# facebookresearch/omni3d

Measured on AMD Instinct MI355X. Metric: images/sec train DLA34_FPN b=4/GPU, higher is better.
Workload: dtype f32; 1 GPU; cubercnn_DLA34_FPN train step, batch 4/GPU, synthetic Omni3D 512x512 (8 GT/img), fwd+10 losses+bwd+allreduce+divergence guard+SGD, random-init weights; global_batch=4, image=512x512, parallelism=dp1 (flat-bucket RCCL all-reduce)

## Files before the change

include/omni3d_hip.h:

```cpp
#ifndef OMNI3D_HIP_H
#define OMNI3D_HIP_H

#ifdef __cplusplus
extern "C" {
#endif


int omni_iou_box3d(const float* boxes1, int N, const float* boxes2, int M, const int* valid1, float* vol,
                   float* iou, int* overflow, void* stream);

int omni_iou_box3d_pairs(const float* boxes1, const float* boxes2, const int* idx1, const int* idx2,
                         long long npairs, const int* valid1, float* vol, float* iou, int* overflow,
                         void* stream);

int omni_iou_box3d_pairs_algo(const float* boxes1, const float* boxes2, const int* idx1, const int* idx2,
                              long long npairs, const int* valid1, float* vol, float* iou, int* overflow,
                              int lanes_per_pair, void* stream);

int omni_box3d_validity(const float* boxes, int N, float eps_coplanar, float eps_nonzero, int* valid,
                        int* counts, void* stream);

int omni_nms3d(const float* verts, const float* score, const int* cls, const int* count, int B, int S, float iou_thr,
               int class_agnostic, float eps_coplanar, float eps_nonzero, float* iou, int* keep, int* order, int* new_count,
               int* overflow, void* stream);
// ... 266 lines not shown
int omni_cuboid_corners(const float* box3d, const float* R, int n, float* verts, void* stream);

int omni_conv2d_fwd_stats(const float* x, const float* w, float* out, int N, int H, int W, int C, int K, int R, int S,
                          int stride, int pad, int ldx, int ldo, float* stats, int stats_rows, int* nblk_out, void* stream);
int omni_wino_out_stats(const float* M, float* y, int N, int H, int W, int K, int tile, float* stats, int stats_rows,
                        int* nblk_out, void* stream);
int omni_wino_out_bn_bwd_stats(const float* M, float* y, int N, int H, int W, int K, int tile, const float* bn_x,
                               const float* mean_rstd, const float* scale_shift, float* stats, int stats_rows, int* nblk_out,
                               void* stream);
int omni_stem_conv_fwd_stats(const float* x, const float* w, float* out, int N, int H, int W, int C, int K, int R, int ldx,
                             int ldo, float* stats, int stats_rows, int* nblk_out, void* stream);

int omni_gemm_engine(const float* A, const float* B, float* C, const float* bias, int form, int batch, int M, int N, int K,
                     int lda, int ldb, int ldc, long long stride_a, long long stride_b, long long stride_c, int splits,
                     int relu, int accumulate, int tile, int workgroups, void* stream);
int omni_gemm_engine_det(const float* A, const float* B, float* C, const float* bias, int form, int batch, int M, int N, int K,
                         int lda, int ldb, int ldc, long long stride_a, long long stride_b, long long stride_c, int splits,
                         int relu, int accumulate, int tile, int workgroups, float* ws, long long ws_floats, int* ctr, int n_ctr,
                         long long* plan, void* stream);

int omni_transpose2d(const float* src, float* dst, int rows, int cols, void* stream);

int omni_det_scores(const float* pred, int ld, const float* rois, const int* count, const int* image_hw, int B, int P, int K,
                    float wx, float wy, float ww, float wh, float score_thresh, float* scores, float* probs, float* boxes,
                    void* stream);
int omni_det_nms_boxes(const float* boxes, const float* vals, const int* idx, int B, int PK, int K, int cap, float* nms_boxes,
                       int* valid, void* stream);
int omni_det_compact(const int* keep, const int* valid, const float* vals, const int* idx, const float* boxes, int B, int PK,
                     int K, int cap, int topk, float* out_box, float* out_score, int* out_cls, int* out_roi, int* out_count,
                     void* stream);

int omni_resize_bilinear_u8(const unsigned char* src, unsigned char* dst, unsigned char* tmp, int planes, int H, int W,
                            int HO, int WO, const int* bounds_h, const int* kk_h, int ksize_h, const int* bounds_v,
                            const int* kk_v, int ksize_v, int flip, void* stream);
int omni_pil_bilinear_coeffs(int in_size, int out_size, int* bounds, int* kk, int ksize, void* stream);
int omni_crop_resize_u8(const unsigned char* src, unsigned char* dst, unsigned char* tmp, int planes, int H, int W, int x0, int y0,
                        int ch, int cw, int HO, int WO, const int* bounds_h, const int* kk_h, int ksize_h, const int* bounds_v,
                        const int* kk_v, int ksize_v, int flip, void* stream);
int omni_color_jitter_u8(unsigned char* img, int H, int W, int wb, int wc, int ws, int c_red, unsigned long long* sum, void* stream);
int omni_warp_homography_u8(const unsigned char* src, unsigned char* dst, int planes, int H, int W, int HO, int WO, const double* m,
                            const unsigned char* fill, void* stream);


int omni_sgd_step(float* param, const float* grad, float* momentum_buf, long long n, float lr, float momentum,
                  float dampening, float weight_decay, int nesterov, int first_step, float grad_scale,
                  const float* skip_flag, void* stream);
int omni_adam_step(float* param, const float* grad, float* exp_avg, float* exp_avg_sq, float* max_exp_avg_sq, long long n, float lr,
                   float beta1, float beta2, float eps, float weight_decay, int decoupled, const float* step, float grad_scale,
                   const float* skip_flag, void* stream);
int omni_adam_tick(float* step, const float* skip_flag, void* stream);
int omni_clip_norm_partials(const float* grad, const long long* tiles, int ntiles, float norm_type, double* partial, void* stream);
int omni_clip_norm_coef(const double* partial, const long long* ptab, int nparams, float norm_type, float max_norm, float grad_scale,
                        float* norm, float* coef, void* stream);
int omni_sgd_step_clipped(float* param, const float* grad, float* momentum_buf, const long long* tiles, int t0, int t1, int clip_mode,
                          const float* coef, float clip_value, float lr, float momentum, float dampening, float weight_decay,
                          int nesterov, int first_step, float grad_scale, const float* skip_flag, void* stream);
int omni_adam_step_clipped(float* param, const float* grad, float* exp_avg, float* exp_avg_sq, float* max_exp_avg_sq,
                           const long long* tiles, int t0, int t1, int clip_mode, const float* coef, float clip_value, float lr,
                           float beta1, float beta2, float eps, float weight_decay, int decoupled, const float* step,
                           float grad_scale, const float* skip_flag, void* stream);
int omni_guard_pre(float* vec, int n, void* stream);
int omni_guard_post(float* vec, int n, int world, float stabilize, float half_period, float tolerance, float gamma, float* state,
                    float* skip, float* out, void* stream);
int omni_scale_vec(const void* src, int src_f64, int stride, const double* coef, const void* denom, double denom_min, int n, float* out,
                   void* stream);
int omni_sum_vectors(const void* const* vecs, const int* lens, int nvec, int nfirst, float* out, void* stream);
int omni_guard_gather(const void* const* scalars, int n, float* vec, void* stream);
int omni_bump_counters(const void* const* counters, int n, long long delta, void* stream);
int omni_zero(void* p, long long nbytes, void* stream);
int omni_nonfinite_any(const float* grad, long long n, float* flag, void* stream);

int omni_relu_bwd(const float* dy, const float* y, float* dz, long long n, void* stream);
int omni_bias_grad(const float* dy, int P, int C, float* db, double* ws, int accumulate, void* stream);

int omni_maxpool3s2_fwd(const float* x, float* y, int N, int H, int W, int C, void* stream);
int omni_maxpool3s2_bwd(const float* x, const float* dy, float* dx, int N, int H, int W, int C, void* stream);

int omni_wino_in(const float* x, float* V, int N, int H, int W, int C, int tile, void* stream);
int omni_wino_out(const float* M, const float* bias, float* y, int N, int H, int W, int K, int relu, int tile, void* stream);
int omni_wino_dy(const float* dy, float* dM, int N, int H, int W, int K, int tile, void* stream);
int omni_wino_weights_multi(const void* const* g, const void* const* U, const void* const* U_flip, const int* K, const int* C,
                            const int* tile, int n, void* stream);
int omni_wino_dy_in(const float* dy, float* dM, float* Vd, int N, int H, int W, int K, int tile, void* stream);
int omni_wino_weights(const float* g, float* U , float* U_flip , int K, int C, int tile, void* stream);
int omni_wino_dweights(const float* dU, float* dg, int K, int C, int accumulate, int tile, void* stream);
int omni_wino_dweights_multi(const void* const* dU, const void* const* dg, const int* K, const int* C, const int* tile, int n,
                             void* stream);
int omni_gemm_batched_fwd_algo(const float* x, const float* w, float* out, int batch, int M, int C, int K, int algo,
                               int workgroups, void* stream);
int omni_gemm_batched_wgrad_algo(const float* x, const float* dy, float* dw, int batch, int M, int C, int K, int algo,
                                 void* stream);
int omni_gemm_batched_wgrad_det(const float* x, const float* dy, float* dw, int batch, int M, int C, int K, int algo, float* ws,
                                long long ws_floats, int* ctr, int n_ctr, long long* plan, void* stream);
int omni_gemm_batched_wgrad_multi(const void* const* x, const void* const* dy, const void* const* dw, const int* batch, const int* M,
                                  const int* C, const int* K, int n, float* ws, long long ws_floats, int* ctr, int n_ctr,
                                  long long* plan, void* stream);

int omni_stem_conv_fwd(const float* x, const float* w, float* out, int N, int H, int W, int C, int K, int R, int ldx, int ldo,
                       void* stream);
int omni_stem_conv_dgrad(const float* dy, const float* w, float* dx, int N, int H, int W, int C, int K, int R, int lddy, int lddx,
                         void* stream);
int omni_stem_conv_s2_dgrad(const float* dy, const float* w, float* dx, int N, int H, int W, int C, int K, int R, int lddy, int lddx,
                            void* stream);
int omni_stem_conv_wgrad(const float* x, const float* dy, float* dw, int N, int H, int W, int C, int K, int R, int ldx, int lddy,
                         int accumulate, void* stream);
int omni_stem_conv_wgrad_det(const float* x, const float* dy, float* dw, int N, int H, int W, int C, int K, int R, int ldx, int lddy,
                             int accumulate, float* ws, long long ws_floats, long long* plan, void* stream);
int omni_stem_conv_fwd_cw(const float* x, const float* w, int cw, float* out, int N, int H, int W, int C, int K, int R, int ldx, int ldo,
                          float* stats, int stats_rows, int* nblk_out, void* stream);
int omni_stem_conv_wgrad_det_cw(const float* x, const float* dy, float* dw, int cw, int N, int H, int W, int C, int K, int R, int ldx,
                                int lddy, int accumulate, float* ws, long long ws_floats, long long* plan, void* stream);
int omni_stem_conv_s2_wgrad(const float* x, const float* dy, float* dw, int N, int H, int W, int C, int K, int R, int ldx, int lddy,
                            int accumulate, int deterministic, float* ws, long long ws_floats, long long* plan, void* stream);

int omni_eval_match(const float* ious, const long long* iou_off, const int* dt_off, const int* gt_off, const int* gt_ignore,
                    const float* gt_range, const float* dt_range, const float* areas, const double* thrs, int ngroups, int A,
                    int T, int sumD, int sumG, int max_gt, int* dt_match, int* gt_match, unsigned char* dt_ignore, int* gt_order,
                    unsigned char* gt_ig, void* stream);

int omni_eval_accumulate(const int* order, const int* cat_off, const int* rank, const double* score, const int* dt_match,
                         const unsigned char* dt_ignore, const int* npig, const int* has_e, const double* rec_thrs,
                         const int* max_dets, int K, int A, int M, int T, int R, int sumD, double* precision, double* recall,
                         double* scores, void* stream);

int omni_eval_accumulate_par_workspace(int K, int A, int M, int T, int sumD, int block, long long* bytes);
int omni_eval_accumulate_par(const int* order, const int* cat_off, const int* rank, const double* score, const int* dt_match,
                             const unsigned char* dt_ignore, const int* npig, const int* has_e, const double* rec_thrs,
                             const int* max_dets, int K, int A, int M, int T, int R, int sumD, int block, void* workspace,
                             long long workspace_bytes, double* precision, double* recall, double* scores, void* stream);

int omni_eval_bootstrap_counts(const int* grp_off, const int* grp_img, const int* grp_npig, const int* weights, int max_weight, int K,
                               int A, int G, int sumG, int B, int I, int* npig_b, int* has_e_b, void* stream);
int omni_eval_bootstrap(const int* order, const int* cat_off, const int* rank, const int* dt_match, const unsigned char* dt_ignore,
                        const int* det_img, const int* weights, int max_weight, const int* npig_b, const int* has_e_b,
                        const double* rec_thrs, const int* max_dets, int K, int A, int M, int T, int R, int sumD, int B, int I,
                        double* ap, double* ar, void* stream);

int omni_eval_error_types(const float* sim, const long long* sim_off, const int* dt_off, const int* gt_off, const int* dt_cat,
                          const unsigned char* dt_matched, const unsigned char* dt_ignore, const double* dt_score, const int* gt_cat,
                          const unsigned char* gt_matched, const unsigned char* gt_ignore, double t_fg, double t_bg, int I, int sumD,
                          int sumG, int max_gt, signed char* type, int* attr, float* smax, unsigned char* win_loc,
                          unsigned char* win_cls, unsigned char* gt_missed, void* stream);

int omni_cuboid_depth(const float* box3d, const float* R, const float* K, int N, int H, int W, float zplane, float* depth,
                      int* index, int* face, int* area, int* visible, void* stream);
int omni_scene_compose(const int* index, const int* face, const float* R, const float* K, const float* color, int N, int H, int W,
                       float blend_weight, unsigned char* image, void* stream);
int omni_draw_segments(const float* seg, int S, unsigned char* image, int H, int W, void* stream);
int omni_fill_shapes(const float* shape, int S, unsigned char* image, int H, int W, void* stream);
int omni_ground_grid(unsigned char* image, const int* index, const float* K, const float* A, const float* t, float y0, int x_start,
                     int x_end, int z_start, int z_end, float near, float thickness, int bg_rgb, int line_rgb, int H, int W,
                     void* stream);

int omni_match_errors(const float* dt_box, const int* dt_cat, const float* dt_c2d, const float* dt_z, const float* dt_dims,
                      const float* dt_pose, const int* dt_off, const float* gt_box, const int* gt_cat, const float* gt_center,
                      const float* gt_dims, const float* gt_pose, const int* gt_off, const float* K, int I, int D, int G, int* match,
                      float* err, double* sums, long long* counts, double* workspace, void* stream);

int omni_train_vis_pick(const float* pred, int ldp, const float* head, int ldh, int uncert_off, const float* rois, const int* cls,
                        const int* nfg, int B, int S, int Fc, int K, float wx, float wy, float ww, float wh, float scale_clamp,
                        float iou_thr, int max_keep, int* keep_row, int* keep_count, float* keep_box, float* keep_score, void* stream);

int omni_box_annotate(const float* box3d, const float* R, const int* box_off, const float* K, const int* size, int I, int N,
                      float min_z, float* verts3d, float* verts2d, float* proj, float* trunc, double* truncation,
                      unsigned char* behind, unsigned char* fully_behind, void* stream);
int omni_visibility_ragged(const float* box3d, const float* R, const int* box_off, const float* K, const int* size,
// ... 32 lines not shown
```

omni3d_amd/csrc/winograd.hip:

```cpp
#include <device_rt.h>

namespace {

__device__ __forceinline__ float4 ld4(const float* p) { return *reinterpret_cast<const float4*>(p); }
__device__ __forceinline__ void st4(float* p, float4 v) { *reinterpret_cast<float4*>(p) = v; }
__device__ __forceinline__ float4 z4() { return make_float4(0.f, 0.f, 0.f, 0.f); }

inline int ew_grid(long total) {
    long g = (total + 255) / 256;
    if (g > 4096) g = 4096;
    return (int)(g < 1 ? 1 : g);
}

__device__ __forceinline__ float4 wino_ld(const float* __restrict__ p, bool ok, bool aff, float4 sc, float4 sh, int relu) {
    if (!ok) return z4();
    float4 v = ld4(p);
    if (aff) {
        v = v * sc + sh;
        if (relu) v = make_float4(fmaxf(v.x, 0.f), fmaxf(v.y, 0.f), fmaxf(v.z, 0.f), fmaxf(v.w, 0.f));
    }
    return v;
}

__global__ void __launch_bounds__(256) wino_in_kernel(const float* __restrict__ x, float* __restrict__ V, int N, int H, int W,
// ... 650 lines not shown
            }
        }
        {
            const float4 g00 = d[1][1], g01 = d[1][2], g10 = d[2][1], g11 = d[2][2];
            float4 u[4][2];
            u[0][0] = g00;        u[0][1] = g01;
            u[1][0] = g00 + g10;  u[1][1] = g01 + g11;
            u[2][0] = g00 - g10;  u[2][1] = g01 - g11;
            u[3][0] = z4() - g10; u[3][1] = z4() - g11;
#pragma unroll
            for (int r = 0; r < 4; ++r) {
                st4(dM + o + (long)(4 * r + 0) * plane, u[r][0]);
                st4(dM + o + (long)(4 * r + 1) * plane, u[r][0] + u[r][1]);
                st4(dM + o + (long)(4 * r + 2) * plane, u[r][0] - u[r][1]);
                st4(dM + o + (long)(4 * r + 3) * plane, z4() - u[r][1]);
            }
        }
    }
}

__global__ void __launch_bounds__(256) wino4_dy_in_kernel(const float* __restrict__ dy, float* __restrict__ dM, float* __restrict__ Vd,
                                                          int N, int H, int W, int K, long plane_in) {
    const int K4 = K >> 2, TH = H >> 2, TW = W >> 2;
    const long T = (long)N * TH * TW, total = T * K4, plane = plane_in > 0 ? plane_in : T * K;
    for (long i = (long)blockIdx.x * blockDim.x + threadIdx.x; i < total; i += (long)gridDim.x * blockDim.x) {
        const int k4 = (int)(i % K4);
        const long t = i / K4;
        const int tx = (int)(t % TW);
        const int ty = (int)((t / TW) % TH);
        const int n = (int)(t / ((long)TW * TH));
        float4 d[6][6];
#pragma unroll
        for (int r = 0; r < 6; ++r) {
            const int ih = 4 * ty - 1 + r;
#pragma unroll
            for (int s = 0; s < 6; ++s) {
                const int iw = 4 * tx - 1 + s;
                const bool ok = (unsigned)ih < (unsigned)H && (unsigned)iw < (unsigned)W;
                d[r][s] = ok ? ld4(dy + (((long)n * H + ih) * W + iw) * K + 4 * k4) : z4();
            }
        }
        const long o = t * K + 4 * k4;
        {
            float4 u[6][4];
#pragma unroll
            for (int c = 0; c < 4; ++c) {
                float4 col[4], o6[6];
#pragma unroll
                for (int r = 0; r < 4; ++r) col[r] = d[1 + r][1 + c];
                a6(col, o6);
#pragma unroll
                for (int r = 0; r < 6; ++r) u[r][c] = o6[r];
            }
#pragma unroll
            for (int r = 0; r < 6; ++r) {
                float4 row[6];
                a6(u[r], row);
#pragma unroll
                for (int c = 0; c < 6; ++c) st4(dM + o + (long)(6 * r + c) * plane, row[c]);
            }
        }
        {
            float4 u[6][6];
#pragma unroll
            for (int s = 0; s < 6; ++s) {
                float4 col[6], tcol[6];
#pragma unroll
                for (int r = 0; r < 6; ++r) col[r] = d[r][s];
                bt6(col, tcol);
#pragma unroll
                for (int r = 0; r < 6; ++r) u[r][s] = tcol[r];
            }
#pragma unroll
            for (int r = 0; r < 6; ++r) {
                float4 v[6];
                bt6(u[r], v);
#pragma unroll
                for (int s = 0; s < 6; ++s) st4(Vd + o + (long)(6 * r + s) * plane, v[s]);
            }
        }
    }
}

inline bool bad(int N, int H, int W, int C) { return N < 0 || H <= 0 || W <= 0 || C <= 0 || (C & 3); }

}

extern "C" {

int omni_wino_in(const float* x, float* V, int N, int H, int W, int C, int tile, void* stream) {
    if (bad(N, H, W, C) || (tile != 2 && tile != 4) || (H % tile) || (W % tile)) return OMNI_ERR_ARG;
    const long total = (long)N * (H / tile) * (W / tile) * (C / 4);
    if (total == 0) return OMNI_OK;
    const float* affine = nullptr;
    const long plane = 0;
    if (tile == 2) hipLaunchKernelGGL(wino_in_kernel, dim3(ew_grid(total)), dim3(256), 0, (hipStream_t)stream, x, V, N, H, W, C, affine, 0, plane);
    else hipLaunchKernelGGL(wino4_in_kernel, dim3(ew_grid(total)), dim3(256), 0, (hipStream_t)stream, x, V, N, H, W, C, affine, 0, plane);
    return omni_launch_status();
}

static int wino_out_impl(const float* M, const float* bias, float* y, int N, int H, int W, int K, int relu, int tile, float* stats,
                         int stats_rows, int* nblk_out, void* stream, BnBwdStats bnb = BnBwdStats{nullptr, nullptr, nullptr},
                         const float* carry = nullptr, long ldc = 0) {
    if (nblk_out) *nblk_out = 0;
    if (bad(N, H, W, K) || (tile != 2 && tile != 4) || (H % tile) || (W % tile)) return OMNI_ERR_ARG;
    const long total = (long)N * (H / tile) * (W / tile) * (K / 4), plane = 0;
    if (total == 0) return OMNI_OK;
    int grid = ew_grid(total);
    float* st_ptr = nullptr;
    if (stats != nullptr && bias == nullptr && !relu && K >= 4 && (256 % (K / 4)) == 0 && (bnb.x == nullptr || tile == 4)) {
        if (grid > stats_rows) grid = stats_rows;
        if (grid >= 1) { st_ptr = stats; if (nblk_out) *nblk_out = grid; }
        else grid = ew_grid(total);
    }
    if (st_ptr == nullptr) bnb = BnBwdStats{nullptr, nullptr, nullptr};
    if (tile == 2) hipLaunchKernelGGL(wino_out_kernel, dim3(grid), dim3(256), 0, (hipStream_t)stream, M, bias, y, N, H, W, K, relu, st_ptr,
                                      carry, ldc, plane);
    else hipLaunchKernelGGL(wino4_out_kernel, dim3(grid), dim3(256), 0, (hipStream_t)stream, M, bias, y, N, H, W, K, relu, st_ptr, bnb,
                            carry, ldc, plane);
    return omni_launch_status();
}

int omni_wino_out(const float* M, const float* bias, float* y, int N, int H, int W, int K, int relu, int tile, void* stream) {
    return wino_out_impl(M, bias, y, N, H, W, K, relu, tile, nullptr, 0, nullptr, stream);
}

int omni_wino_out_carry(const float* M, const float* carry, long long ldc, float* y, int N, int H, int W, int K, int tile, void* stream) {
    if (carry == nullptr || ldc < K || (ldc & 3) || (((unsigned long long)carry) & 15)) return OMNI_ERR_ARG;
    return wino_out_impl(M, nullptr, y, N, H, W, K, 0, tile, nullptr, 0, nullptr, stream, BnBwdStats{nullptr, nullptr, nullptr}, carry, (long)ldc);
}

int omni_wino_out_bn_bwd_stats(const float* M, float* y, int N, int H, int W, int K, int tile, const float* bn_x, const float* mean_rstd,
                               const float* scale_shift, float* stats, int stats_rows, int* nblk_out, void* stream) {
    if (bn_x == nullptr || mean_rstd == nullptr) return OMNI_ERR_ARG;
    return wino_out_impl(M, nullptr, y, N, H, W, K, 0, tile, stats, stats_rows, nblk_out, stream, BnBwdStats{bn_x, mean_rstd, scale_shift});
}

int omni_wino_out_stats(const float* M, float* y, int N, int H, int W, int K, int tile, float* stats, int stats_rows, int* nblk_out,
                        void* stream) {
    return wino_out_impl(M, nullptr, y, N, H, W, K, 0, tile, stats, stats_rows, nblk_out, stream);
}

int omni_wino_dy(const float* dy, float* dM, int N, int H, int W, int K, int tile, void* stream) {
    if (bad(N, H, W, K) || (tile != 2 && tile != 4) || (H % tile) || (W % tile)) return OMNI_ERR_ARG;
    const long total = (long)N * (H / tile) * (W / tile) * (K / 4);
    if (total == 0) return OMNI_OK;
    if (tile == 2) hipLaunchKernelGGL(wino_dy_kernel, dim3(ew_grid(total)), dim3(256), 0, (hipStream_t)stream, dy, dM, N, H, W, K);
    else hipLaunchKernelGGL(wino4_dy_kernel, dim3(ew_grid(total)), dim3(256), 0, (hipStream_t)stream, dy, dM, N, H, W, K);
    return omni_launch_status();
}

int omni_wino_dy_in(const float* dy, float* dM, float* Vd, int N, int H, int W, int K, int tile, void* stream) {
    if (bad(N, H, W, K) || (tile != 2 && tile != 4) || (H % tile) || (W % tile)) return OMNI_ERR_ARG;
    const long total = (long)N * (H / tile) * (W / tile) * (K / 4), plane = 0;
    if (total == 0) return OMNI_OK;
    if (tile == 2) hipLaunchKernelGGL(wino_dy_in_kernel, dim3(ew_grid(total)), dim3(256), 0, (hipStream_t)stream, dy, dM, Vd, N, H, W, K, plane);
    else hipLaunchKernelGGL(wino4_dy_in_kernel, dim3(ew_grid(total)), dim3(256), 0, (hipStream_t)stream, dy, dM, Vd, N, H, W, K, plane);
    return omni_launch_status();
}

int omni_wino_weights(const float* g, float* U, float* U_flip, int K, int C, int tile, void* stream) {
    if (K <= 0 || C <= 0 || (U == nullptr && U_flip == nullptr) || (tile != 2 && tile != 4)) return OMNI_ERR_ARG;
    const unsigned wt = (unsigned)wino4_w_tiles(K, C);
    if (tile == 2) hipLaunchKernelGGL(wino_w_kernel, dim3(wt), dim3(256), 0, (hipStream_t)stream, g, U, U_flip, K, C);
    else hipLaunchKernelGGL(wino4_w_kernel, dim3(wt), dim3(256), 0, (hipStream_t)stream, g, U, U_flip, K, C);
    return omni_launch_status();
}

int omni_wino_weights_multi(const void* const* g, const void* const* U, const void* const* U_flip, const int* K, const int* C,
                            const int* tile, int n, void* stream) {
    if (n <= 0 || n > WINO_MULTI_MAX || g == nullptr || U == nullptr || U_flip == nullptr) return OMNI_ERR_ARG;
    WinoWTable t;
    t.n = n;
    t.wg0[0] = 0;
    for (int i = 0; i < n; ++i) {
        if (K[i] <= 0 || C[i] <= 0 || (U[i] == nullptr && U_flip[i] == nullptr) || (tile[i] != 2 && tile[i] != 4) || g[i] == nullptr)
            return OMNI_ERR_ARG;
        t.g[i] = (const float*)g[i];
        t.U[i] = (float*)U[i];
        t.Uf[i] = (float*)U_flip[i];
        t.K[i] = K[i]; t.C[i] = C[i]; t.tile[i] = tile[i];
        t.wg0[i + 1] = t.wg0[i] + wino4_w_tiles(K[i], C[i]);
    }
    hipLaunchKernelGGL(wino_w_multi_kernel, dim3((unsigned)t.wg0[n]), dim3(256), 0, (hipStream_t)stream, t);
    return omni_launch_status();
}

int omni_wino_dweights(const float* dU, float* dg, int K, int C, int accumulate, int tile, void* stream) {
    if (K <= 0 || C <= 0 || (tile != 2 && tile != 4)) return OMNI_ERR_ARG;
    if (tile == 2) hipLaunchKernelGGL(wino_dw_kernel, dim3(ew_grid((long)K * C)), dim3(256), 0, (hipStream_t)stream, dU, dg, K, C, accumulate);
    else hipLaunchKernelGGL(wino4_dw_kernel, dim3(ew_grid((long)K * C)), dim3(256), 0, (hipStream_t)stream, dU, dg, K, C, accumulate);
    return omni_launch_status();
}

int omni_wino_dweights_multi(const void* const* dU, const void* const* dg, const int* K, const int* C, const int* tile, int n, void* stream) {
    if (n <= 0 || n > WINO_DW_MAX || dU == nullptr || dg == nullptr) return OMNI_ERR_ARG;
    WinoDwTable t;
    int dest[WINO_DW_MAX], nd = 0;
    for (int i = 0; i < n; ++i) {
        if (K[i] <= 0 || C[i] <= 0 || (tile[i] != 2 && tile[i] != 4) || dU[i] == nullptr || dg[i] == nullptr) return OMNI_ERR_ARG;
        int d = 0;
        while (d < nd && t.dg[d] != (float*)dg[i]) ++d;
        if (d == nd) {
            t.dg[nd] = (float*)dg[i]; t.K[nd] = K[i]; t.C[nd] = C[i];
            ++nd;
        } else if (t.K[d] != K[i] || t.C[d] != C[i]) {
            return OMNI_ERR_ARG;
        }
        dest[i] = d;
    }
    t.n = nd;
    t.wg0[0] = 0;
    int q = 0;
    for (int d = 0; d < nd; ++d) {
        t.src0[d] = q;
        for (int i = 0; i < n; ++i)
            if (dest[i] == d) { t.dU[q] = (const float*)dU[i]; t.tile[q] = tile[i]; ++q; }
        const long wgs = ((long)t.K[d] * t.C[d] + 255) / 256;
        if (t.wg0[d] + wgs > 0x7fffffff) return OMNI_ERR_ARG;
        t.wg0[d + 1] = t.wg0[d] + (int)wgs;
    }
    t.src0[nd] = q;
    hipLaunchKernelGGL(wino_dw_multi_kernel, dim3((unsigned)t.wg0[nd]), dim3(256), 0, (hipStream_t)stream, t);
    return omni_launch_status();
}

}
```

omni3d_amd/kernels/wino.py:

```python
import torch

from .. import lib as _lib
from . import detmode as _det

CL = torch.channels_last


import os as _os

_F43_MIN_TILES = 256
_MIN_TILES = 256
_DGRAD_MIN_TILES = 256


def eligible(x_shape, w_shape, stride, pad):
    N, C, H, W = x_shape
    K, _, R, S = w_shape
    if not (R == 3 and S == 3 and stride == 1 and pad == 1 and H % 2 == 0 and W % 2 == 0 and C % 32 == 0 and K % 32 == 0):
        return False
    if C >= 128 and K >= 128 and N * (H // 2) * (W // 2) >= _MIN_TILES:
        return True
    return C >= 64 and K >= 64 and tile_size(x_shape) == 4 and N * (H // 4) * (W // 4) >= 4096


# ... 185 lines not shown
    if _deferred is None or not _multi_fits(V, dM):
        return transform_dweights(gemm_batched_wgrad(V, dM), accum_into)
    _deferred.append((V, dM, accum_into))
    return None


def transform_output(Mt, shape, bias=None, relu=False, carry=None):
    tile = 2 if Mt.shape[0] == 16 else 4
    N, H, W = shape
    K = Mt.shape[2]
    L = _lib.check_device(Mt, bias)
    y = torch.empty((N, H, W, K), dtype=torch.float32, device=Mt.device)
    if carry is not None:
        assert bias is None and not relu and tuple(carry.shape) == (N, K, H, W)
        L.call("omni_wino_out_carry", _lib.ptr(Mt), carry.data_ptr(), carry.stride(3), _lib.ptr(y), N, H, W, K, tile, _lib.stream_of(Mt))
        return y.permute(0, 3, 1, 2)
    L.call("omni_wino_out", _lib.ptr(Mt), _lib.ptr(bias), _lib.ptr(y), N, H, W, K, int(relu), tile, _lib.stream_of(Mt))
    return y.permute(0, 3, 1, 2)


def transform_output_stats(Mt, shape):
    from .conv import STATS_ROWS, _nblk_cell, _stats_buf
    tile = 2 if Mt.shape[0] == 16 else 4
    N, H, W = shape
    K = Mt.shape[2]
    L = _lib.check_device(Mt)
    y = torch.empty((N, H, W, K), dtype=torch.float32, device=Mt.device)
    stats = _stats_buf(K, Mt.device)
    cell, addr = _nblk_cell()
    L.call("omni_wino_out_stats", _lib.ptr(Mt), _lib.ptr(y), N, H, W, K, tile, _lib.ptr(stats), STATS_ROWS, addr, _lib.stream_of(Mt))
    return y.permute(0, 3, 1, 2), (stats[:cell.value] if cell.value > 0 else None)


def transform_output_bn_bwd(Mt, shape, bn_x, mean_rstd, scale_shift):
    from .conv import STATS_ROWS, _nblk_cell, _stats_buf
    tile = 2 if Mt.shape[0] == 16 else 4
    N, H, W = shape
    K = Mt.shape[2]
    xv = bn_x.permute(0, 2, 3, 1)
    assert xv.is_contiguous() and tuple(xv.shape) == (N, H, W, K)
    L = _lib.check_device(Mt, xv, mean_rstd, scale_shift)
    y = torch.empty((N, H, W, K), dtype=torch.float32, device=Mt.device)
    stats = _stats_buf(K, Mt.device)
    cell, addr = _nblk_cell()
    L.call("omni_wino_out_bn_bwd_stats", _lib.ptr(Mt), _lib.ptr(y), N, H, W, K, tile, _lib.ptr(xv), _lib.ptr(mean_rstd), _lib.ptr(scale_shift),
           _lib.ptr(stats), STATS_ROWS, addr, _lib.stream_of(Mt))
    return y.permute(0, 3, 1, 2), (stats[:cell.value] if cell.value > 0 else None)


def transform_dy(dy, tile=2):
    dv = _nhwc(dy)
    N, H, W, K = dv.shape
    L = _lib.check_device(dv)
    dM = torch.empty((_points(tile), N * (H // tile) * (W // tile), K), dtype=torch.float32, device=dy.device)
    L.call("omni_wino_dy", _lib.ptr(dv), _lib.ptr(dM), N, H, W, K, tile, _lib.stream_of(dy))
    return dM


def transform_dy_both(dy, tile=2):
    dv = _nhwc(dy)
    N, H, W, K = dv.shape
    L = _lib.check_device(dv)
    shape = (_points(tile), N * (H // tile) * (W // tile), K)
    dM = torch.empty(shape, dtype=torch.float32, device=dy.device)
    Vd = torch.empty(shape, dtype=torch.float32, device=dy.device)
    L.call("omni_wino_dy_in", _lib.ptr(dv), _lib.ptr(dM), _lib.ptr(Vd), N, H, W, K, tile, _lib.stream_of(dy))
    return dM, Vd


def transform_dweights(dU, accum_into=None):
    P, K, C = dU.shape
    tile = 2 if P == 16 else 4
    L = _lib.check_device(dU)
    if accum_into is not None:
        gv = accum_into.permute(0, 2, 3, 1)
        assert gv.is_contiguous()
        L.call("omni_wino_dweights", _lib.ptr(dU), _lib.ptr(gv), K, C, 1, tile, _lib.stream_of(dU))
        return None
    dw = torch.empty((K, 3, 3, C), dtype=torch.float32, device=dU.device)
    L.call("omni_wino_dweights", _lib.ptr(dU), _lib.ptr(dw), K, C, 0, tile, _lib.stream_of(dU))
    return dw.permute(0, 3, 1, 2)


def conv3x3_fwd(x, w, bias=None, relu=False, U=None, tile=2, want_stats=False):
    N, _, H, W = x.shape
    V = transform_input(x, tile)
    if U is None:
        U = transform_weights(w, tile=tile)[0]
    Mt = gemm_batched(V, U)
    if want_stats:
        y, parts = transform_output_stats(Mt, (N, H, W))
        return y, V, parts
    return transform_output(Mt, (N, H, W), bias, relu), V


def conv3x3_dgrad(dy, w, U_flip=None, tile=2, carry=None):
    N, _, H, W = dy.shape
    if U_flip is None:
        U_flip = transform_weights(w, want_u=False, want_flip=True, tile=tile)[1]
    Mt = gemm_batched(transform_input(dy, tile), U_flip)
    return transform_output(Mt, (N, H, W), carry=carry)


def conv3x3_backward(V, dy, w, U_flip, accum_into=None, side_run=None, bn_below=None, carry=None):
    N, _, H, W = dy.shape
    tile = 2 if V.shape[0] == 16 else 4
    dM, Vd = transform_dy_both(dy, tile)
    if side_run is not None and accum_into is not None:
        dw = side_run(lambda: wgrad_into(V, dM, accum_into), (V, dM))
    else:
        dw = None
    if U_flip is None:
        U_flip = transform_weights(w, want_u=False, want_flip=True, tile=tile)[1]
    if carry is not None:
        dx = transform_output(gemm_batched(Vd, U_flip), (N, H, W), carry=carry)
    elif bn_below is not None and tile == 4:
        dx, parts = transform_output_bn_bwd(gemm_batched(Vd, U_flip), (N, H, W), *bn_below[:3])
        if parts is not None:
            dx._omni_bn_bwd_parts = (parts, bn_below[1])
    else:
        dx = transform_output(gemm_batched(Vd, U_flip), (N, H, W))
    if side_run is None or accum_into is None:
        dw = transform_dweights(gemm_batched_wgrad(V, dM), accum_into)
    return dx, dw


def conv3x3_wgrad(V, dy, accum_into=None):
    dM = transform_dy(dy, 2 if V.shape[0] == 16 else 4)
    if accum_into is not None:
        return wgrad_into(V, dM, accum_into)
    return transform_dweights(gemm_batched_wgrad(V, dM), None)
```

omni3d_amd/profile_io.py:

```python
import csv
import hashlib
import os
import re

ROOT = os.path.dirname(os.path.dirname(os.path.abspath(__file__)))


def profile_counters(csv_name, kernel_substr, grid=None):
    path = os.path.join(ROOT, "profiles", csv_name)
    if not os.path.exists(path):
        return None
    digest = hashlib.sha256(open(path, "rb").read()).hexdigest()[:16]
    rows = [r for r in csv.DictReader(open(path)) if kernel_substr in r["kernel"] and (grid is None or int(float(r["grid"])) == grid)]
    if not rows:
        return None
    r = max(rows, key=lambda q: float(q.get("GRBM_GUI_ACTIVE", "0") or 0))

    def f(k):
        try:
            v = float(r[k])
            return v if v == v else None
        except (KeyError, ValueError):
            return None
    out = {"source": f"profiles/{csv_name}", "sha256_16": digest, "kernel": r["kernel"], "grid": int(float(r["grid"]))}
# ... 3 lines not shown
    if out["SQ_VALU_MFMA_BUSY_CYCLES"] and out["GRBM_GUI_ACTIVE"]:
        out["mfma_busy_frac"] = out["SQ_VALU_MFMA_BUSY_CYCLES"] / (out["GRBM_GUI_ACTIVE"] / 8.0 * 1024.0)
    if out["SQ_ACTIVE_INST_VALU"] and out["SQ_WAVE_CYCLES"]:
        out["valu_active_frac_of_wave_cycles"] = out["SQ_ACTIVE_INST_VALU"] / out["SQ_WAVE_CYCLES"]
    if out["SQ_ACTIVE_INST_VALU"] and out["GRBM_GUI_ACTIVE"]:
        out["valu_busy_frac_of_simd_cycles"] = out["SQ_ACTIVE_INST_VALU"] * 4.0 / (out["GRBM_GUI_ACTIVE"] / 8.0 * 1024.0)
    if out.get("SQ_THREAD_CYCLES_VALU") and out["SQ_INSTS_VALU"]:
        out["valu_lane_utilisation"] = out["SQ_THREAD_CYCLES_VALU"] / (64.0 * out["SQ_INSTS_VALU"])
    return out


def latest_profile(name, rounds=("r06", "r05", "r04", "r03", "r02")):
    for r in rounds:
        if os.path.exists(os.path.join(ROOT, "profiles", f"{r}_{name}")):
            return f"{r}_{name}"
    return f"{rounds[0]}_{name}"


class ExecutedFlops:

    def __enter__(self):
        from . import lib
        self.lib = lib.get()
        self.flops = 0.0
        self.by_entry = {}
        self._orig = self.lib.call

        def call(name, *a):
            f = self._flops(name, a)
            if f:
                self.flops += f
                self.by_entry[name] = self.by_entry.get(name, 0.0) + f
            return self._orig(name, *a)
        self.lib.call = call
        return self

    def __exit__(self, *exc):
        self.lib.call = self._orig
        return False

    @staticmethod
    def _flops(name, a):
        return executed_flops(name, a)


_SIGNATURES = None
MFMA_ENTRY = re.compile(r"conv|gemm|stem|head16")
VALU_ENTRIES = frozenset(["omni_dwconv_fwd", "omni_dwconv_dgrad", "omni_dwconv_wgrad", "omni_rpn_head16_dgrad", "omni_rpn_head16_wgrad"])


def abi_signatures():
    global _SIGNATURES
    if _SIGNATURES is None:
        text = re.sub(r"/\*.*?\*/", "", open(os.path.join(ROOT, "include", "omni3d_hip.h")).read(), flags=re.S)
        _SIGNATURES = {m.group(1): [x.strip().split()[-1].lstrip("*") for x in " ".join(m.group(2).split()).split(",")]
                       for m in re.finditer(r"\bint\s+(omni_\w+)\s*\(([^)]*)\)\s*;", text)}
    return _SIGNATURES


def flop_class(name):
    names = abi_signatures().get(name)
    if names is None or not MFMA_ENTRY.search(name):
        return None
    if name in VALU_ENTRIES:
        return "valu"
    if name.startswith("omni_rpn_head16"):
        return "head16"
    if name.startswith("omni_stem_conv"):
        return "stem"
    if name.startswith("omni_gemm_engine"):
        return "engine"
    if name == "omni_gemm_batched_wgrad_multi":
        return "gemm_batched_multi"
    if name.startswith("omni_gemm_batched"):
        return "gemm_batched"
    if name.startswith("omni_grouped_conv2d"):
        return "grouped"
    if name in ("omni_conv2d_fwd_multi_det", "omni_conv2d_wgrad_multi_det"):
        return "conv_multi"
    if name == "omni_conv2d_s2_dgrad":
        return "conv_s2"
    if name.startswith("omni_conv2d"):
        return "conv"
    return None


def _host_ints(ptr, n, ctype):
    import ctypes
    if ptr is None:
        return []
    addr = ptr.value if hasattr(ptr, "value") else int(ptr)
    return list(ctypes.cast(addr, ctypes.POINTER(ctype))[:n])


def executed_flops(name, a):
    import ctypes
    cls = flop_class(name)
    if cls in (None, "valu"):
        return 0.0
    v = dict(zip(abi_signatures()[name], a))
    if v.get("plan") is not None:
        return 0.0
    if cls in ("conv", "grouped"):
        OH = (v["H"] + 2 * v["pad"] - v["R"]) // v["stride"] + 1
        OW = (v["W"] + 2 * v["pad"] - v["S"]) // v["stride"] + 1
        return 2.0 * v["N"] * OH * OW * v["K"] * v["R"] * v["S"] * v["C"] / (v["groups"] if cls == "grouped" else 1)
    if cls == "conv_multi":
        return 2.0 * v["N"] * v["H"] * v["W"] * v["K"] * sum(_host_ints(v["cs"], v["nsrc"], ctypes.c_int))
    if cls == "conv_s2":
        return 2.0 * v["N"] * ((v["H"] - 1) // 2 + 1) * ((v["W"] - 1) // 2 + 1) * v["K"] * 9 * v["C"]
    if cls == "stem":
        stride = 2 if "_s2_" in name else 1
        OH, OW = (v["H"] - 1) // stride + 1, (v["W"] - 1) // stride + 1
        return 2.0 * v["N"] * OH * OW * v["K"] * v["R"] * v["R"] * v["C"]
    if cls == "gemm_batched":
        if "N" in v and "C" not in v:
            return 2.0 * v["batch"] * v["M"] * v["N"] * v["K"]
        return 2.0 * v["batch"] * v["M"] * v["C"] * v["K"]
    if cls == "gemm_batched_multi":
        n = v["n"]
        cols = [_host_ints(v[k], n, ctypes.c_int) for k in ("batch", "M", "C", "K")]
        return float(sum(2.0 * b * m * c * k for b, m, c, k in zip(*cols)))
    if cls == "engine":
        return 2.0 * v["batch"] * v["M"] * v["N"] * v["K"]
    if cls == "head16":
        return 2.0 * sum(_host_ints(v["pix"], v["nlev"], ctypes.c_longlong)) * 256 * 16
    return 0.0


def host_cores():
    import os
    info = {"logical_cpus": os.cpu_count(), "affinity_cpus": len(os.sched_getaffinity(0)) if hasattr(os, "sched_getaffinity") else None,
            "physical_cores": None, "sockets": None, "model": None}
    try:
        cores, pk = set(), None
        for line in open("/proc/cpuinfo"):
            if line.startswith("physical id"):
                pk = line.split(":")[1].strip()
            elif line.startswith("core id"):
                cores.add((pk, line.split(":")[1].strip()))
            elif line.startswith("model name") and info["model"] is None:
                info["model"] = line.split(":")[1].strip()
        if cores:
            info["physical_cores"] = len(cores)
            info["sockets"] = len({c[0] for c in cores})
    except OSError:
        pass
    return info


class GpuState:

    FILES = (("sclk_mhz", "freq1_input", 1e-6), ("mclk_mhz", "freq2_input", 1e-6), ("power_w", "power1_input", 1e-6),
             ("temp_junction_c", "temp2_input", 1e-3), ("temp_mem_c", "temp3_input", 1e-3))

    def __init__(self, index=0):
        self.dir, self.hwmon, self.address = None, None, None
        try:
            import glob
            import torch
            p = torch.cuda.get_device_properties(index)
            self.address = "%04x:%02x:%02x.0" % (p.pci_domain_id, p.pci_bus_id, p.pci_device_id)
            d = os.path.join("/sys/bus/pci/devices", self.address)
            hw = sorted(glob.glob(os.path.join(d, "hwmon", "hwmon*")))
            if hw:
                self.dir, self.hwmon = d, hw[0]
        except Exception:
            pass

    @staticmethod
    def _read(path, scale):
        try:
            with open(path) as f:
                return round(float(f.read().split()[0]) * scale, 1)
        except (OSError, ValueError, IndexError):
            return None

    def sample(self):
        if self.hwmon is None:
            return None
        out = {k: self._read(os.path.join(self.hwmon, f), s) for k, f, s in self.FILES}
        out["busy_pct"] = self._read(os.path.join(self.dir, "gpu_busy_percent"), 1.0)
        return out

    def neighbours(self):
        if self.hwmon is None:
            return None
        import glob
        n = up = 0
        watts = 0.0
        for hw in glob.glob("/sys/bus/pci/devices/*/hwmon/hwmon*"):
            if hw == self.hwmon:
                continue
            try:
                if open(os.path.join(hw, "name")).read().strip() != "amdgpu":
                    continue
            except OSError:
# ... 7 lines not shown
```

Baseline: 381.8 images/s.

## Fuse Winograd F(4,3) input transform, MFMA GEMM and output transform for 64-channel convs

Adds one kernel for 3x3 convs with 64 input and 64 output channels that does the Winograd input transform into LDS, the 36 batched 16x16x4 MFMA products against the transformed weights, and the output transform with bias/ReLU/BN-stats or carry/BN-backward epilogues. The 64-channel forward and dgrad paths now use it instead of separate transform, GEMM and output-transform kernels. The goal is to skip writing the transformed tiles to global memory and reading them back, and to cut launches. It still writes V/dM to global for the weight-gradient GEMM. It is specialised to C=K=64, and its 16-tile blocks with large LDS use may limit occupancy compared with the tuned generic GEMM.

After: 383.8 images/s (median of 6 runs). Within noise of the previous version (+0.5%).

```diff
diff --git a/include/omni3d_hip.h b/include/omni3d_hip.h
--- a/include/omni3d_hip.h
+++ b/include/omni3d_hip.h
@@ -372,6 +372,11 @@
 int omni_wino_weights_multi(const void* const* g, const void* const* U, const void* const* U_flip, const int* K, const int* C,
                             const int* tile, int n, void* stream);
 int omni_wino_dy_in(const float* dy, float* dM, float* Vd, int N, int H, int W, int K, int tile, void* stream);
+int omni_wino4_conv64_fwd(const float* x, const float* U, const float* bias, float* V, float* y, int N, int H, int W, int C, int K,
+                          int relu, float* stats, int stats_rows, int* nblk_out, void* stream);
+int omni_wino4_conv64_bwd(const float* dy, const float* U_flip, float* dM, float* dx, int N, int H, int W, int C, int K,
+                          const float* carry, long long ldc, const float* bn_x, const float* mean_rstd, const float* scale_shift,
+                          float* stats, int stats_rows, int* nblk_out, void* stream);
 int omni_wino_weights(const float* g, float* U , float* U_flip , int K, int C, int tile, void* stream);
 int omni_wino_dweights(const float* dU, float* dg, int K, int C, int accumulate, int tile, void* stream);
 int omni_wino_dweights_multi(const void* const* dU, const void* const* dg, const int* K, const int* C, const int* tile, int n,
diff --git a/omni3d_amd/csrc/winograd.hip b/omni3d_amd/csrc/winograd.hip
--- a/omni3d_amd/csrc/winograd.hip
+++ b/omni3d_amd/csrc/winograd.hip
@@ -756,7 +756,232 @@
     }
 }
 
+constexpr int F64_TB = 16;
+constexpr int F64_LD = 68;
+constexpr int F64_LDS_BYTES = 36 * F64_TB * F64_LD * 4;
+constexpr int F64_MAX_ROWS = 512;
+
+struct Fused64Epi {
+    const float* bias;
+    int relu;
+    float* stats;
+    BnBwdStats bnb;
+    const float* carry;
+    long ldc;
+};
+
+__device__ __forceinline__ f32x4 f64_point(const float4 (&a)[4], const float4 (&b)[4]) {
+    f32x4 c0 = {0.f, 0.f, 0.f, 0.f}, c1 = {0.f, 0.f, 0.f, 0.f};
+    c0 = mfma_16x16x4(a[0].x, b[0].x, c0); c1 = mfma_16x16x4(a[2].x, b[2].x, c1);
+    c0 = mfma_16x16x4(a[0].y, b[0].y, c0); c1 = mfma_16x16x4(a[2].y, b[2].y, c1);
+    c0 = mfma_16x16x4(a[0].z, b[0].z, c0); c1 = mfma_16x16x4(a[2].z, b[2].z, c1);
+    c0 = mfma_16x16x4(a[0].w, b[0].w, c0); c1 = mfma_16x16x4(a[2].w, b[2].w, c1);
+    c0 = mfma_16x16x4(a[1].x, b[1].x, c0); c1 = mfma_16x16x4(a[3].x, b[3].x, c1);
+    c0 = mfma_16x16x4(a[1].y, b[1].y, c0); c1 = mfma_16x16x4(a[3].y, b[3].y, c1);
+    c0 = mfma_16x16x4(a[1].z, b[1].z, c0); c1 = mfma_16x16x4(a[3].z, b[3].z, c1);
+    c0 = mfma_16x16x4(a[1].w, b[1].w, c0); c1 = mfma_16x16x4(a[3].w, b[3].w, c1);
+    return c0 + c1;
+}
+
+template <bool BWD>
+__global__ void __launch_bounds__(256) wino4_conv64_kernel(const float* __restrict__ x, const float* __restrict__ U,
+                                                           float* __restrict__ Vout, float* __restrict__ y, int N, int H, int W,
+                                                           Fused64Epi e) {
+    HIP_DYNAMIC_SHARED(float, s_v)
+    constexpr int C = 64;
+    const int TH = H >> 2, TW = W >> 2;
+    const long T = (long)N * TH * TW, plane = T * C, nblk = (T + F64_TB - 1) / F64_TB;
+    const int lane = threadIdx.x & 63, wv = threadIdx.x >> 6, r = lane & 15, q = lane >> 4;
+    const int k = 16 * wv + r;
+    const unsigned ub = (unsigned)(k * C + 4 * q);
+    const float* ab = s_v + r * F64_LD + 4 * q;
+    float sv = 0.f, sq = 0.f;
+    float mu = 0.f, rs = 0.f, sc = 0.f, sh = 0.f;
+    if (BWD && e.bnb.x != nullptr) {
+        mu = e.bnb.mean_rstd[k]; rs = e.bnb.mean_rstd[C + k];
+        if (e.bnb.scale_shift != nullptr) { sc = e.bnb.scale_shift[k]; sh = e.bnb.scale_shift[C + k]; }
+    }
+    const float bias = (!BWD && e.bias != nullptr) ? e.bias[k] : 0.f;
+    for (long blk = blockIdx.x; blk < nblk; blk += gridDim.x) {
+        const long tb0 = blk * F64_TB;
+        {
+            const int tl = threadIdx.x >> 4, c4 = threadIdx.x & 15;
+            const long t = tb0 + tl;
+            const bool live = t < T;
+            const int tx = (int)(t % TW), ty = (int)((t / TW) % TH), n = live ? (int)(t / ((long)TW * TH)) : 0;
+            float4 d[6][6];
+#pragma unroll
+            for (int rr = 0; rr < 6; ++rr) {
+                const int ih = 4 * ty - 1 + rr;
+#pragma unroll
+                for (int s = 0; s < 6; ++s) {
+                    const int iw = 4 * tx - 1 + s;
+                    const bool ok = live && (unsigned)ih < (unsigned)H && (unsigned)iw < (unsigned)W;
+                    d[rr][s] = wino_ld(x + (((long)n * H + ih) * W + iw) * C + 4 * c4, ok, false, z4(), z4(), 0);
+                }
+            }
+            const long o = t * C + 4 * c4;
+            if (BWD && live) {
+                float4 u[6][4];
+#pragma unroll
+                for (int c = 0; c < 4; ++c) {
+                    float4 col[4], o6[6];
+#pragma unroll
+                    for (int rr = 0; rr < 4; ++rr) col[rr] = d[1 + rr][1 + c];
+                    a6(col, o6);
+#pragma unroll
+                    for (int rr = 0; rr < 6; ++rr) u[rr][c] = o6[rr];
+                }
+#pragma unroll
+                for (int rr = 0; rr < 6; ++rr) {
+                    float4 row[6];
+                    a6(u[rr], row);
+#pragma unroll
+                    for (int c = 0; c < 6; ++c) st4(Vout + o + (long)(6 * rr + c) * plane, row[c]);
+                }
+            }
+            float4 u[6][6];
+#pragma unroll
+            for (int s = 0; s < 6; ++s) {
+                float4 col[6], tcol[6];
+#pragma unroll
+                for (int rr = 0; rr < 6; ++rr) col[rr] = d[rr][s];
+                bt6(col, tcol);
+#pragma unroll
+                for (int rr = 0; rr < 6; ++rr) u[rr][s] = tcol[rr];
+            }
+            float* sp = s_v + tl * F64_LD + 4 * c4;
+#pragma unroll
+            for (int rr = 0; rr < 6; ++rr) {
+                float4 v[6];
+                bt6(u[rr], v);
+#pragma unroll
+                for (int s = 0; s < 6; ++s) {
+                    st4(sp + (6 * rr + s) * (F64_TB * F64_LD), v[s]);
+                    if (!BWD && live) st4(Vout + o + (long)(6 * rr + s) * plane, v[s]);
+                }
+            }
+        }
+        OMNI_SCHED_FENCE();
+        float4 b[3][4], a[2][4];
+        {
+            unsigned pofs = 0;
+            OMNI_OPAQUE_S(pofs);
+            const float* up = U + (pofs + ub);
+#pragma unroll
+            for (int j = 0; j < 4; ++j) { b[0][j] = ld4(up + 16 * j); b[1][j] = ld4(up + 4096 + 16 * j); }
+        }
+        __syncthreads();
+        f32x4 acc[36];
+#pragma unroll
+        for (int j = 0; j < 4; ++j) a[0][j] = ld4(ab + 16 * j);
+        OMNI_SCHED_FENCE();
+#pragma unroll
+        for (int p = 0; p < 36; ++p) {
+            if (p + 2 < 36) {
+                unsigned pofs = (p + 2) * 4096;
+                OMNI_OPAQUE_S(pofs);
+                const float* up = U + (pofs + ub);
+#pragma unroll
+                for (int j = 0; j < 4; ++j) b[(p + 2) % 3][j] = ld4(up + 16 * j);
+            }
+            if (p + 1 < 36) {
+#pragma unroll
+                for (int j = 0; j < 4; ++j) a[(p + 1) & 1][j] = ld4(ab + (p + 1) * (F64_TB * F64_LD) + 16 * j);
+            }
+            acc[p] = f64_point(a[p & 1], b[p % 3]);
+            OMNI_SCHED_FENCE();
+        }
+#pragma unroll
+        for (int i = 0; i < 4; ++i) {
+            const long t = tb0 + 4 * q + i;
+            if (t < T) {
+                const int tx = (int)(t % TW), ty = (int)((t / TW) % TH), n = (int)(t / ((long)TW * TH));
+                float s[4][6];
+#pragma unroll
+                for (int c = 0; c < 6; ++c) {
+                    float col[6], o4[4];
+#pragma unroll
+                    for (int rr = 0; rr < 6; ++rr) col[rr] = acc[6 * rr + c][i];
+                    at6(col, o4);
+#pragma unroll
+                    for (int rr = 0; rr < 4; ++rr) s[rr][c] = o4[rr];
+                }
+#pragma unroll
+                for (int rr = 0; rr < 4; ++rr) {
+                    float row[4];
+                    at6(s[rr], row);
+                    const long pix = ((long)n * H + 4 * ty + rr) * W + 4 * tx;
+                    const long off = pix * C + k;
+                    if (BWD && e.carry != nullptr) {
+                        float cv[4];
+#pragma unroll
+                        for (int c = 0; c < 4; ++c) cv[c] = e.carry[(pix + c) * e.ldc + k];
+#pragma unroll
+                        for (int c = 0; c < 4; ++c) y[off + (long)c * C] = row[c] + cv[c];
+                    } else if (BWD && e.bnb.x != nullptr) {
+                        float xv[4];
+#pragma unroll
+                        for (int c = 0; c < 4; ++c) xv[c] = e.bnb.x[off + (long)c * C];
+#pragma unroll
+                        for (int c = 0; c < 4; ++c) {
+                            const float v = row[c];
+                            y[off + (long)c * C] = v;
+                            float g = v;
+                            if (e.bnb.scale_shift != nullptr) g = (xv[c] * sc + sh) > 0.f ? v : 0.f;
+                            const float xh = (xv[c] - mu) * rs;
+                            sv = sv + g;
+                            sq = sq + g * xh;
+                        }
+                    } else {
+#pragma unroll
+                        for (int c = 0; c < 4; ++c) {
+                            float v = row[c] + bias;
+                            if (!BWD && e.relu) v = fmaxf(v, 0.f);
+                            y[off + (long)c * C] = v;
+                            sv = sv + v;
+                            sq = sq + v * v;
+                        }
+                    }
+                }
+            }
+        }
+        __syncthreads();
+    }
+    if (e.stats != nullptr) {
+        sv += __shfl_xor(sv, 16, 64); sq += __shfl_xor(sq, 16, 64);
+        sv += __shfl_xor(sv, 32, 64); sq += __shfl_xor(sq, 32, 64);
+        if (q == 0) {
+            e.stats[(long)blockIdx.x * 2 * C + k] = sv;
+            e.stats[(long)blockIdx.x * 2 * C + C + k] = sq;
+        }
+    }
+}
+
 inline bool bad(int N, int H, int W, int C) { return N < 0 || H <= 0 || W <= 0 || C <= 0 || (C & 3); }
+
+template <bool BWD>
+int conv64_launch(const float* x, const float* U, float* Vout, float* y, int N, int H, int W, Fused64Epi e, int stats_rows, int* nblk_out,
+                  void* stream) {
+    if (nblk_out) *nblk_out = 0;
+    const long T = (long)N * (H / 4) * (W / 4);
+    if (T == 0) return OMNI_OK;
+    long grid = (T + F64_TB - 1) / F64_TB;
+    if (grid > 0x7fffffffL) return OMNI_ERR_ARG;
+    if (e.stats != nullptr) {
+        const int cap = stats_rows < F64_MAX_ROWS ? stats_rows : F64_MAX_ROWS;
+        if (cap < 1) return OMNI_ERR_ARG;
+        if (grid > cap) grid = cap;
+        if (nblk_out) *nblk_out = (int)grid;
+    }
+#ifndef OMNI_HIPEMU
+    static const hipError_t lds_ok = hipFuncSetAttribute(reinterpret_cast<const void*>(&wino4_conv64_kernel<BWD>),
+                                                         hipFuncAttributeMaxDynamicSharedMemorySize, F64_LDS_BYTES);
+    if (lds_ok != hipSuccess) return OMNI_ERR_LAUNCH;
+#endif
+    hipLaunchKernelGGL(wino4_conv64_kernel<BWD>, dim3((unsigned)grid), dim3(256), F64_LDS_BYTES, (hipStream_t)stream, x, U, Vout, y, N, H, W, e);
+    return omni_launch_status();
+}
 
 }
 
@@ -899,4 +1124,26 @@
     return omni_launch_status();
 }
 
-}
+int omni_wino4_conv64_fwd(const float* x, const float* U, const float* bias, float* V, float* y, int N, int H, int W, int C, int K,
+                          int relu, float* stats, int stats_rows, int* nblk_out, void* stream) {
+    if (nblk_out) *nblk_out = 0;
+    if (bad(N, H, W, C) || C != 64 || K != 64 || (H & 3) || (W & 3) || x == nullptr || U == nullptr || V == nullptr || y == nullptr)
+        return OMNI_ERR_ARG;
+    Fused64Epi e{bias, relu, stats, BnBwdStats{nullptr, nullptr, nullptr}, nullptr, 0};
+    return conv64_launch<false>(x, U, V, y, N, H, W, e, stats_rows, nblk_out, stream);
+}
+
+int omni_wino4_conv64_bwd(const float* dy, const float* U_flip, float* dM, float* dx, int N, int H, int W, int C, int K,
+                          const float* carry, long long ldc, const float* bn_x, const float* mean_rstd, const float* scale_shift,
+                          float* stats, int stats_rows, int* nblk_out, void* stream) {
+    if (nblk_out) *nblk_out = 0;
+    if (bad(N, H, W, C) || C != 64 || K != 64 || (H & 3) || (W & 3) || dy == nullptr || U_flip == nullptr || dM == nullptr || dx == nullptr)
+        return OMNI_ERR_ARG;
+    if (carry != nullptr && (bn_x != nullptr || ldc < K || (ldc & 3) || (((unsigned long long)carry) & 15))) return OMNI_ERR_ARG;
+    if (bn_x != nullptr && (mean_rstd == nullptr || stats == nullptr)) return OMNI_ERR_ARG;
+    if (bn_x == nullptr && stats != nullptr) return OMNI_ERR_ARG;
+    Fused64Epi e{nullptr, 0, stats, BnBwdStats{bn_x, mean_rstd, scale_shift}, carry, (long)ldc};
+    return conv64_launch<true>(dy, U_flip, dM, dx, N, H, W, e, stats_rows, nblk_out, stream);
+}
+
+}
diff --git a/omni3d_amd/kernels/wino.py b/omni3d_amd/kernels/wino.py
--- a/omni3d_amd/kernels/wino.py
+++ b/omni3d_amd/kernels/wino.py
@@ -291,11 +291,58 @@
     return dw.permute(0, 3, 1, 2)
 
 
+FUSED64 = True
+
+
+def fused64_eligible(x_shape, K, tile):
+    return FUSED64 and tile == 4 and x_shape[1] == 64 and K == 64 and x_shape[2] % 4 == 0 and x_shape[3] % 4 == 0
+
+
+def conv64_fwd(x, U, bias=None, relu=False, want_stats=False):
+    from .conv import STATS_ROWS, _nblk_cell, _stats_buf
+    xv = _nhwc(x)
+    N, H, W, C = xv.shape
+    K = U.shape[1]
+    L = _lib.check_device(xv, U, bias)
+    V = torch.empty((36, N * (H // 4) * (W // 4), C), dtype=torch.float32, device=x.device)
+    y = torch.empty((N, H, W, K), dtype=torch.float32, device=x.device)
+    stats = _stats_buf(K, x.device) if want_stats else None
+    cell, addr = _nblk_cell()
+    L.call("omni_wino4_conv64_fwd", _lib.ptr(xv), _lib.ptr(U), _lib.ptr(bias), _lib.ptr(V), _lib.ptr(y), N, H, W, C, K, int(relu),
+           _lib.ptr(stats), STATS_ROWS, addr, _lib.stream_of(x))
+    return y.permute(0, 3, 1, 2), V, (stats[:cell.value] if cell.value > 0 else None)
+
+
+def conv64_bwd(dy, U_flip, carry=None, bn_below=None):
+    from .conv import STATS_ROWS, _nblk_cell, _stats_buf
+    dv = _nhwc(dy)
+    N, H, W, K = dv.shape
+    C = U_flip.shape[1]
+    dM = torch.empty((36, N * (H // 4) * (W // 4), K), dtype=torch.float32, device=dy.device)
+    dx = torch.empty((N, H, W, C), dtype=torch.float32, device=dy.device)
+    bn_x = mean_rstd = scale_shift = stats = None
+    if carry is not None:
+        assert bn_below is None and tuple(carry.shape) == (N, C, H, W)
+    elif bn_below is not None:
+        bn_x, mean_rstd, scale_shift = bn_below[0].permute(0, 2, 3, 1), bn_below[1], bn_below[2]
+        assert bn_x.is_contiguous() and tuple(bn_x.shape) == (N, H, W, C)
+        stats = _stats_buf(C, dy.device)
+    L = _lib.check_device(dv, U_flip, bn_x, mean_rstd, scale_shift)
+    cell, addr = _nblk_cell()
+    L.call("omni_wino4_conv64_bwd", _lib.ptr(dv), _lib.ptr(U_flip), _lib.ptr(dM), _lib.ptr(dx), N, H, W, C, K,
+           None if carry is None else carry.data_ptr(), 0 if carry is None else carry.stride(3), _lib.ptr(bn_x), _lib.ptr(mean_rstd),
+           _lib.ptr(scale_shift), _lib.ptr(stats), STATS_ROWS, addr, _lib.stream_of(dy))
+    return dx.permute(0, 3, 1, 2), dM, (stats[:cell.value] if cell.value > 0 else None)
+
+
 def conv3x3_fwd(x, w, bias=None, relu=False, U=None, tile=2, want_stats=False):
     N, _, H, W = x.shape
-    V = transform_input(x, tile)
     if U is None:
         U = transform_weights(w, tile=tile)[0]
+    if fused64_eligible(x.shape, w.shape[0], tile):
+        y, V, parts = conv64_fwd(x, U, bias, relu, want_stats)
+        return (y, V, parts) if want_stats else (y, V)
+    V = transform_input(x, tile)
     Mt = gemm_batched(V, U)
     if want_stats:
         y, parts = transform_output_stats(Mt, (N, H, W))
@@ -314,13 +361,20 @@
 def conv3x3_backward(V, dy, w, U_flip, accum_into=None, side_run=None, bn_below=None, carry=None):
     N, _, H, W = dy.shape
     tile = 2 if V.shape[0] == 16 else 4
+    if U_flip is None:
+        U_flip = transform_weights(w, want_u=False, want_flip=True, tile=tile)[1]
+    if fused64_eligible(dy.shape, w.shape[1], tile):
+        dx, dM, parts = conv64_bwd(dy, U_flip, carry=carry, bn_below=None if carry is not None or bn_below is None else bn_below[:3])
+        if parts is not None:
+            dx._omni_bn_bwd_parts = (parts, bn_below[1])
+        if side_run is not None and accum_into is not None:
+            return dx, side_run(lambda: wgrad_into(V, dM, accum_into), (V, dM))
+        return dx, transform_dweights(gemm_batched_wgrad(V, dM), accum_into)
     dM, Vd = transform_dy_both(dy, tile)
     if side_run is not None and accum_into is not None:
         dw = side_run(lambda: wgrad_into(V, dM, accum_into), (V, dM))
     else:
         dw = None
-    if U_flip is None:
-        U_flip = transform_weights(w, want_u=False, want_flip=True, tile=tile)[1]
     if carry is not None:
         dx = transform_output(gemm_batched(Vd, U_flip), (N, H, W), carry=carry)
     elif bn_below is not None and tile == 4:
diff --git a/omni3d_amd/profile_io.py b/omni3d_amd/profile_io.py
--- a/omni3d_amd/profile_io.py
+++ b/omni3d_amd/profile_io.py
@@ -109,6 +109,8 @@
         return "conv_s2"
     if name.startswith("omni_conv2d"):
         return "conv"
+    if name.startswith("omni_wino4_conv64"):
+        return "wino_fused"
     return None
 
 
@@ -140,6 +142,8 @@
         stride = 2 if "_s2_" in name else 1
         OH, OW = (v["H"] - 1) // stride + 1, (v["W"] - 1) // stride + 1
         return 2.0 * v["N"] * OH * OW * v["K"] * v["R"] * v["R"] * v["C"]
+    if cls == "wino_fused":
+        return 2.0 * 36 * v["N"] * (v["H"] // 4) * (v["W"] // 4) * v["C"] * v["K"]
     if cls == "gemm_batched":
         if "N" in v and "C" not in v:
             return 2.0 * v["batch"] * v["M"] * v["N"] * v["K"]
```
